# latentnetworks/vimure

Measured on AMD Instinct MI355X. Metric: CAVI iterations/sec (L=4 N=2000 M=200 K=2 synthetic, mutuality on), higher is better.
Workload: dtype f64

## Files before the change

vimure_amd/csrc/sweep_sl.hip:

```cpp
#include "sweep_sl.h"

#ifndef VMR_K
#error "compile with -DVMR_K=<number of categories>"
#endif
#ifndef SL_WPE
#define SL_WPE sl_wpe(2, false, true)
#endif

template <int K>
struct StepIn {
  double v[K];
  double w[K];
  unsigned cls, qt, tie;
  unsigned x0;
  unsigned e[sl_pf(K)];
};

template <int R> struct RC { static constexpr int value = R; };
template <class V> __device__ __forceinline__ const V* at_bytes(const V* p, unsigned off) {
  return reinterpret_cast<const V*>(reinterpret_cast<const char*>(p) + off);
}
template <class V> __device__ __forceinline__ V* at_bytes(V* p, unsigned off) {
  return reinterpret_cast<V*>(reinterpret_cast<char*>(p) + off);
}
__device__ __forceinline__ double rcp_nr2(double d) {
  double r = __builtin_amdgcn_rcp(d);
  r = fma(fma(-d, r, 1.0), r, r);
  return fma(fma(-d, r, 1.0), r, r);
}
#define SL_INL __attribute__((always_inline))
#ifndef SL_BATCH2
#define SL_BATCH2 8
#endif
template <int K> struct Batch { static constexpr int value = K <= 2 ? SL_BATCH2 : (K <= 4 ? 4 : 2); };

template <int K, bool UPDATE, bool ELBO, bool ALLFULL, bool STORE = true, bool DET = false, bool LPD = false>
__device__ __forceinline__ void sweep_body(const SlArgs& a, const Geo& g, const unsigned bx, const unsigned gx) {
  extern __shared__ __align__(16) unsigned char smem[];
  constexpr int PFK = sl_pf(K);
  constexpr bool LV0 = !UPDATE && !ELBO && !DET;
  constexpr bool LV0R = UPDATE && K >= 3;
  const int tid = threadIdx.x, lane = tid & 63, nthr = (int)blockDim.x;
  const int wv = __builtin_amdgcn_readfirstlane(tid >> 6), nw = nthr >> 6;
  const int Mp = g.Mp;
  const unsigned ytm = UPDATE ? (unsigned)a.yt * (unsigned)Mp : 0u;
  const unsigned hcm = a.do_hist ? (unsigned)a.hc * (unsigned)Mp : 0u;
  size_t off = 0;
  double* F = reinterpret_cast<double*>(smem + off); off += (size_t)ytm * K * 8;
  const int nHc = (int)hcm * K;
  double* Hc = reinterpret_cast<double*>(smem + off); off += (size_t)nHc * 8;
  double* Gth = reinterpret_cast<double*>(smem + off); off += (size_t)Mp * 8;
  double* Lth = reinterpret_cast<double*>(smem + off); off += UPDATE ? (size_t)Mp * 8 : 0;
  double* As = reinterpret_cast<double*>(smem + off); off += a.sum_a ? (size_t)Mp * K * 8 : 0;
  double* wsum = reinterpret_cast<double*>(smem + off); off += (size_t)g.W * 8;
  double* red = reinterpret_cast<double*>(smem + off); off += 16 * 8;
  double* xt = reinterpret_cast<double*>(smem + off); off += 64 * 8;
  double* lt = reinterpret_cast<double*>(smem + off); off += ELBO ? 256 * 8 : 0;
  double* EthL = reinterpret_cast<double*>(smem + off); off += a.rq ? (size_t)Mp * 8 : 0;
  const ParOff o = par_off(g.L, g.Mp, g.K);
  const int l = (int)bx / a.Gl, gb = (int)bx - l * a.Gl;
#ifdef SL_DEBUG
  unsigned long long* dbt = a.dbg_t ? a.dbg_t + ((size_t)bx * nw + wv) * 8 : nullptr;
  if (dbt && lane == 0) dbt[0] = wall_clock64();
#endif
  const size_t T = (size_t)g.N * g.N;
  const long long NS = (long long)((T + 63) / 64);
  const double gnu = a.par[o.sc + ((UPDATE || a.elbo_cur) ? SC_G_NU : SC_G_NU_STALE)];
  bool gz = false;
  for (int m = tid; m < Mp; m += nthr) {
    const double gv = a.par[o.G_th + (size_t)l * Mp + m];
    Gth[m] = gv;
    if (LV0 || LV0R) gz = gz || (m < g.M && gv == 0.0);
    if (UPDATE) Lth[m] = a.par[o.l_th + (size_t)l * Mp + m];
  }
  for (int q = tid; q < nHc; q += nthr) Hc[q] = 0.0;
  if (a.sum_a) for (int q = tid; q < Mp * K; q += nthr) As[q] = 0.0;
  if (a.rq) for (int m = tid; m < Mp; m += nthr) EthL[m] = m < g.M ? a.par[o.E_th + (size_t)l * Mp + m] : 0.0;
  if (UPDATE || ELBO) sp_math_tables(xt, lt, tid, nthr, ELBO);
  const double* lut = a.lutg + (size_t)l * g.W * 256;
  for (int w = tid; w < g.W; w += nthr) {
    double v = 0.0;
    for (int n = 0; n < 16; ++n) v += lut[(w * 16 + n) * 16 + 15];
    wsum[w] = v;
  }
  double Ela[K], Gla[K], Lla[K];
#pragma unroll
  for (int k = 0; k < K; ++k) { Ela[k] = a.par[o.E_la + l * K + k]; Gla[k] = a.par[o.G_la + l * K + k]; Lla[k] = a.par[o.l_la + l * K + k]; if (LV0 || LV0R) gz = gz || Gla[k] == 0.0; }
  const double eps = g.eps;
  const double sc_h = DET ? __builtin_amdgcn_ldexp(1.0, g.det_sh) : 0.0, sc_r = DET ? __builtin_amdgcn_ldexp(1.0, g.det_shr) : 0.0;
  const double sc_a = DET ? __builtin_amdgcn_ldexp(1.0, DET_SH_A) : 0.0;
  auto fxm = [](double v, double scale) SL_INL -> unsigned long long {
    return (unsigned long long)(__double_as_longlong(fma(v, scale, 6755399441055744.0)) - 0x4338000000000000ll);
  };
  auto lds_add = [&](double* p, double v, double scale) SL_INL {
    if (DET) atomicAdd(reinterpret_cast<unsigned long long*>(p), fxm(v, scale)); else atomicAdd(p, v);
  };
  const float rcp_mp = 1.0f / (float)Mp, hrcp_mp = 0.5f * rcp_mp;
  auto row_level = [&](unsigned ym) SL_INL -> unsigned { return (unsigned)__builtin_fmaf((float)ym, rcp_mp, hrcp_mp); };
  const double lp0_0 = log(1.0 + eps), lp0_k = log(eps);
  double e_lin = 0.0, e_q = 0.0, e_log = 0.0;
  double accF[K], acc0[K];
#pragma unroll
  for (int k = 0; k < K; ++k) { accF[k] = 0.0; acc0[k] = 0.0; }
  unsigned long long ie_lin = 0ull, ie_q = 0ull, ie_log = 0ull, iaccF[K];
#pragma unroll
  for (int k = 0; k < K; ++k) iaccF[k] = 0ull;
  double* Hl = a.Hg + ((size_t)l * NH + (gb % NH)) * g.Y * Mp * K;
  auto det_H = [&]() SL_INL { return a.det + (size_t)l * g.Y * Mp * K; };
  auto det_A = [&]() SL_INL { return a.det + (size_t)g.L * g.Y * Mp * K + (size_t)l * g.W * 64 * K; };
  auto det_F = [&]() SL_INL { return a.det + (size_t)g.L * g.Y * Mp * K + (size_t)g.L * g.W * 64 * K + (size_t)l * K; };
  auto det_R = [&]() SL_INL { return a.det + (size_t)g.L * g.Y * Mp * K + (size_t)g.L * g.W * 64 * K + (size_t)g.L * K; };
  const unsigned* rsl = a.rs + (size_t)l * (NS + 1);
  const unsigned* syl = a.sy + (size_t)l * NS;
  const unsigned* El = a.E + a.ebase[l];
  const unsigned* pl = (a.rm2 ? a.rm2 : a.perm) + (size_t)l * NS * 64;
  const uint8_t* cl = ALLFULL ? nullptr : a.cls + (size_t)l * T;
  const unsigned* Ql = a.Qt ? a.Qt + (size_t)l * T : nullptr;
  const uint64_t* Rl = a.Rb ? a.Rb + (size_t)l * T * g.W : nullptr;
  double* rl = a.rho + (size_t)l * T * K;
  double* rho_slack = a.rho + (size_t)g.L * T * K;
  const double* lpl = a.logpr + (size_t)l * T * K;
  constexpr bool LPDV = LPD && K == 2 && UPDATE && !ELBO;
  const double* lpdl = LPDV ? a.lpd + (size_t)l * T : nullptr;
  const double lpb0 = (K == 2 && UPDATE) ? a.lpb[2 * l] : 0.0, lpb1 = (K == 2 && UPDATE) ? a.lpb[2 * l + 1] : 0.0;
  const unsigned* rql = a.rq ? a.rq + (size_t)l * (T + 1) : nullptr;
  const unsigned short* Rml = a.rq ? a.Rm + a.rbase[l] : nullptr;
  const unsigned lim_y = UPDATE ? (a.do_hist ? (unsigned)min(a.yt, a.hc) : (unsigned)a.yt) : (a.do_hist ? (unsigned)a.hc : 0xffffffffu);
  const unsigned lim1 = (UPDATE && a.yt < g.Y) ? (unsigned)a.yt : 0xffffffffu;
  const unsigned lim2 = (a.do_hist && a.hc < g.Y) ? (unsigned)a.hc : 0xffffffffu;

  const long long Gl_ = a.Gl;
  unsigned* tick = reinterpret_cast<unsigned*>(smem + off); off += 16;
  if (tid == 0) { tick[0] = 2u * (unsigned)nw; tick[1] = 0u; }
  auto step_of = [&](unsigned t) SL_INL -> long long { return (long long)gb + (long long)t * Gl_; };
  auto draw = [&]() SL_INL -> long long {
    unsigned t = 0u;
    if (lane == 0) t = atomicAdd(tick, 1u);
    return step_of((unsigned)__builtin_amdgcn_readfirstlane((int)t));
  };
  long long s = step_of((unsigned)wv), sn = step_of((unsigned)(nw + wv));
  unsigned ea = 0;
  int R = 0;
  unsigned ymax = 0;
  unsigned rgv = 0;
  StepIn<K> P;

  const unsigned lane4 = (unsigned)lane * 4u, laneK8 = (unsigned)lane * (unsigned)(K * 8);
  const unsigned T32 = (unsigned)T;
  auto fetch_range = [&](long long st) SL_INL {
    const unsigned ra = rsl[st + (lane < 1 ? 0 : 1)], ry = syl[st];
    rgv = lane == 2 ? ry : ra;
  };
  auto fetch_tie = [&](StepIn<K>& d, long long st, const bool lp_const = false) SL_INL {
    const size_t row0 = (size_t)st * 64;
    const bool ok = (unsigned)row0 + (unsigned)lane < T32;
    d.qt = 0u; d.tie = 0u;
    if (ALLFULL) d.cls = ok ? 1u : 0u;
    else {
      const unsigned c = (unsigned)*at_bytes(cl + row0, (unsigned)lane);
      d.cls = ok ? c : 0u;
      d.tie = *at_bytes(pl + row0, lane4);
    }
    if (ELBO && Ql) d.qt = *at_bytes(Ql + row0, lane4);
    d.x0 = 0u;
    if (LV0 && a.x0p) d.x0 = *at_bytes(a.x0p + (size_t)l * NS * 64 + row0, lane4);
#pragma unroll
    for (int k = 0; k < K; ++k) { d.v[k] = 0.0; d.w[k] = 0.0; }
    if (LPDV) {
      if (lp_const) d.v[0] = lp0_k - lp0_0;
      else d.v[0] = *at_bytes(lpdl + row0, (unsigned)lane * 8u);
    } else if (UPDATE || ELBO) {
      if (lp_const) {
#pragma unroll
        for (int k = 0; k < K; ++k) d.v[k] = k == 0 ? lp0_0 : lp0_k;
      } else load_k<K>(at_bytes(lpl + row0 * K, laneK8), d.v);
    }
    if (!UPDATE && a.do_hist != 2) load_k<K>(at_bytes(static_cast<const double*>(rl) + row0 * K, laneK8), d.w);
  };
  auto fetch_ent = [&](StepIn<K>& d, unsigned base, auto cntc) SL_INL {
    constexpr int CNT = decltype(cntc)::value;
    const unsigned* pe = El + base;
#pragma unroll
    for (int j = 0; j < CNT; ++j) d.e[j] = *at_bytes(pe + j * 64, lane4);
  };

  if (s < NS) {
    ea = rsl[s];
    R = (int)((rsl[s + 1] - ea) >> 6);
    ymax = syl[s];
    fetch_range(sn < NS ? sn : s);
    fetch_tie(P, s);
    fetch_ent(P, ea, RC<PFK>{});
  }
#ifdef SL_DEBUG
  if (dbt && lane == 0) dbt[4] = wall_clock64();
#endif
  __builtin_amdgcn_s_waitcnt(0x0F70);
  bool lv0_off = false;
  if (LV0 || LV0R) lv0_off = __syncthreads_or(gz ? 1 : 0) != 0;
  else __syncthreads();
#ifdef SL_DEBUG
  if (dbt && lane == 0) dbt[5] = wall_clock64();
#endif
  const double gnu_f = a.par[o.sc + (a.nu_stale ? SC_G_NU_STALE : SC_G_NU)];
  if (UPDATE) {
    for (int q = tid; q < (int)ytm; q += nthr) {
      const int y = q / Mp, m = q - y * Mp;
#pragma unroll
      for (int k = 0; k < K; ++k) F[q * K + k] = (m < g.M) ? f_entry(g.mut, Lth[m], Gth[m], Lla[k], Gla[k], gnu_f, y) : 0.0;
    }
    __syncthreads();
  }
  double Tfull = 0.0;
  for (int w = 0; w < g.W; ++w) Tfull += wsum[w];
#ifdef SL_DEBUG
  if (dbt && lane == 0) dbt[1] = wall_clock64();
#endif

  auto add_lists = [&](unsigned t, bool on, const double (&rr)[K]) SL_INL {
    if (a.rm2) {
#pragma unroll
      for (int h_ = 0; h_ < 2; ++h_) {
        const unsigned m = h_ ? (t >> 16) : (t & 0xffffu);
        const bool v = on && m != 0xffffu;
        const unsigned long long vm = __ballot(v);
        if (vm == 0ull) continue;
        const int m0 = __builtin_amdgcn_readlane((int)m, __builtin_ctzll(vm));
        if (__all(!v || (int)m == m0)) {
#pragma unroll
          for (int k = 0; k < K; ++k) {
            const double sm_ = wave_sum(v ? rr[k] : 0.0);
            if (lane == 0) lds_add(&As[m0 * K + k], sm_, sc_a);
          }
        } else if (v) {
#pragma unroll
          for (int k = 0; k < K; ++k) lds_add(&As[m * K + k], rr[k], sc_a);
        }
      }
      return;
    }
    unsigned q0 = 0, q1 = 0;
    if (on) { q0 = rql[t]; q1 = rql[t + 1]; }
    for (unsigned i = 0;; ++i) {
      const bool v = q0 + i < q1;
      const unsigned long long vm = __ballot(v);
      if (vm == 0ull) break;
      const int m = v ? (int)Rml[q0 + i] : -1;
      const int m0 = __builtin_amdgcn_readlane(m, __builtin_ctzll(vm));
      if (__all(!v || m == m0)) {
#pragma unroll
        for (int k = 0; k < K; ++k) {
          const double sm_ = wave_sum(v ? rr[k] : 0.0);
          if (lane == 0) lds_add(&As[m0 * K + k], sm_, sc_a);
        }
      } else if (v) {
#pragma unroll
        for (int k = 0; k < K; ++k) lds_add(&As[m * K + k], rr[k], sc_a);
      }
    }
  };
  auto mask_sum = [&](unsigned cls, unsigned tie) SL_INL -> double {
    if (ALLFULL) return Tfull;
    double Tt = 0.0;
    if (cls == 1u) Tt = Tfull;
    else if (cls == 2u && a.rm2) {
      const unsigned m0 = tie & 0xffffu, m1 = tie >> 16;
      Tt = (m0 != 0xffffu ? EthL[m0] : 0.0) + (m1 != 0xffffu ? EthL[m1] : 0.0);
    } else if (cls == 2u && rql) {
      const unsigned q0 = rql[tie], q1 = rql[tie + 1];
      for (unsigned q = q0; q < q1; ++q) Tt += EthL[Rml[q]];
    } else if (cls == 2u) {
      const uint64_t* rwt = Rl + (size_t)tie * g.W;
      for (int w = 0; w < g.W; ++w) {
        uint64_t bits = rwt[w];
        if (bits == ~0ull) { Tt += wsum[w]; continue; }
        for (int n = 0; bits != 0; ++n, bits >>= 4) Tt += lut[((w * 16 + n) << 4) + (unsigned)(bits & 15u)];
      }
    }
    return Tt;
  };
  const double gnu_cur = a.par[o.sc + SC_G_NU];
  auto w2_at = [&](unsigned ym, int k) SL_INL -> double {
    const unsigned y = row_level(ym);
    const double z2 = gnu_cur * (double)y, den = Gth[ym - y * (unsigned)Mp] * Gla[k] + z2;
    return (y == 0u || den == 0.0) ? 0.0 : z2 / den;
  };
  auto f_far = [&](unsigned ym, double (&f)[K]) SL_INL {
    const unsigned y = row_level(ym);
    const unsigned m = ym - y * (unsigned)Mp;
    const double lt = Lth[m], gt = Gth[m];
#pragma unroll
    for (int k = 0; k < K; ++k) f[k] = f_entry(g.mut, lt, gt, Lla[k], Gla[k], gnu_f, (int)y);
  };
  auto elbo_inner = [&](unsigned ent, const double (&er)[2]) SL_INL -> double {
    const unsigned ym = SL_YM(ent);
    const unsigned y = row_level(ym);
    const double z2 = gnu * (double)y, gt = Gth[ym - y * (unsigned)Mp];
    const double inner = fma(gt, er[0], z2 * er[1]);
    return (SL_INR(ent) ? inner : 0.0) + eps;
  };
  auto walk1_near = [&](const unsigned* e, auto npc, double (&U)[K]) SL_INL {
    constexpr int NP = decltype(npc)::value, BT = Batch<K>::value;
#pragma unroll
    for (int j0 = 0; j0 < NP; j0 += BT) {
      double f[BT][K];
#pragma unroll
      for (int u = 0; u < BT; ++u) {
        if (j0 + u < NP) {
#pragma unroll
          for (int k = 0; k < K; ++k) f[u][k] = F[SL_YM(e[j0 + u]) * K + k];
        }
      }
#pragma unroll
      for (int u = 0; u < BT; ++u) {
        if (j0 + u < NP) {
          const double dx = (double)SL_X(e[j0 + u]);
#pragma unroll
          for (int k = 0; k < K; ++k) U[k] = fma(dx, f[u][k], U[k]);
        }
      }
    }
  };
  auto walk2_near = [&](const unsigned* e, auto npc, const double (&r)[K], const double (&er)[2]) SL_INL {
#ifndef SL_LG
#define SL_LG 2
#endif
    constexpr int NP = decltype(npc)::value, LG = SL_LG;
#pragma unroll
    for (int j0 = 0; j0 < NP; j0 += LG) {
      double in_[LG];
#pragma unroll
      for (int u = 0; u < LG; ++u) {
        if (j0 + u < NP) {
          const unsigned ym = SL_YM(e[j0 + u]);
          const double dx = (double)SL_X(e[j0 + u]);
          if (a.do_hist) {
#pragma unroll
            for (int k = 1; k < K; ++k) lds_add(&Hc[(unsigned)k * hcm + ym], dx * r[k], sc_h);
          }
          if (ELBO) in_[u] = elbo_inner(e[j0 + u], er);
        }
      }
      if (ELBO) {
#pragma unroll
        for (int u = 0; u < LG; ++u) if (j0 + u < NP) {
          const double term = (double)SL_X(e[j0 + u]) * log_tab(in_[u], lt);
          if (DET) ie_log += fxm(term, sc_r); else e_log += term;
        }
        __builtin_amdgcn_sched_barrier(0);
      }
    }
  };
  auto deficit = [&](unsigned ent, double dfc) SL_INL {
    lds_add(&Hc[SL_YM(ent)], (double)SL_X(ent) * dfc, sc_h);
  };
  auto compute = [&](auto rct, const StepIn<K>& cur, const size_t row0, const bool act, const unsigned ea_c, const int Rr, const unsigned sy_word) SL_INL {
    const unsigned ymax = sy_word & 0xffffu, nf = a.farl ? sy_word >> 16 : 0x7fffffffu;
    const unsigned n1 = (LV0 && a.h0s && !lv0_off) ? sy_word >> 16 : 0x7fffffffu;
    constexpr int RCT = decltype(rct)::value;
    constexpr int NP = RCT < 0 ? PFK : RCT;
    const unsigned cls = cur.cls, qt = cur.qt, tie = cur.tie;
    const unsigned* pe = El + ea_c;
    auto rounds = [&](auto gbc, auto&& use, const int Rr) SL_INL {
      constexpr int GB = decltype(gbc)::value;
      unsigned rg[PFK];
#pragma unroll
      for (int i = 0; i < PFK; ++i) rg[i] = i < Rr ? cur.e[i] : 0u;
      for (int j0 = 0; j0 < Rr; j0 += PFK) {
#pragma unroll
        for (int gi = 0; gi < PFK; gi += GB) {
          unsigned c[GB];
#pragma unroll
          for (int u = 0; u < GB; ++u) {
            c[u] = rg[gi + u];
            const int jn = j0 + gi + u + PFK;
            rg[gi + u] = *at_bytes(jn < Rr ? pe + (size_t)jn * 64 : a.Ez, lane4);
          }
          if (j0 + gi < Rr) use(c, (unsigned)(j0 + gi));
        }
      }
    };
    double r[K], er[2] = {0.0, 0.0};
#pragma unroll
    for (int k = 0; k < K; ++k) r[k] = act ? cur.w[k] : 0.0;
    if (a.do_hist == 2) {
#pragma unroll
      for (int k = 0; k < K; ++k) r[k] = (k == 1) ? 1.0 : 0.0;
    }
    double Tt = 0.0;
    if (UPDATE || ELBO) Tt = mask_sum(cls, tie);
    double dfc = 0.0;
    bool irr = false;

    if (UPDATE) {
      double U[K];
#pragma unroll
      for (int k = 0; k < K; ++k) U[k] = 0.0;
#ifdef SL_DEBUG
      if (g.dbg & 16) {} else
#endif
      if (RCT >= 0) walk1_near(cur.e, RC<NP>{}, U);
      else {
        constexpr int GB = Batch<K>::value < 4 ? Batch<K>::value : 4;
        const unsigned n1u = (LV0R && a.lv0r && !lv0_off) ? sy_word >> 16 : 0x7fffffffu;
        double sl0 = 0.0, sx1 = 0.0;
        rounds(RC<GB>{}, [&](const unsigned (&c)[GB], const unsigned j) SL_INL {
          if (LV0R && j >= n1u) {
            double l0[GB];
#pragma unroll
            for (int u = 0; u < GB; ++u) l0[u] = Lth[SL_YM(c[u])];
#pragma unroll
            for (int u = 0; u < GB; ++u) { const double dx = (double)SL_X(c[u]); sl0 = fma(dx, l0[u], sl0); sx1 += dx; }
            return;
          }
          if (ymax < lim1 || j >= nf) { walk1_near(c, RC<GB>{}, U); return; }
          double f[GB][K];
          bool fr[GB];
#pragma unroll
          for (int u = 0; u < GB; ++u) {
            const unsigned ym = SL_YM(c[u]);
            fr[u] = ym >= ytm;
#pragma unroll
            for (int k = 0; k < K; ++k) f[u][k] = F[(fr[u] ? 0u : ym) * K + k];
          }
#pragma unroll
          for (int u = 0; u < GB; ++u) {
            const double dx = fr[u] ? 0.0 : (double)SL_X(c[u]);
#pragma unroll
            for (int k = 0; k < K; ++k) U[k] = fma(dx, f[u][k], U[k]);
          }
#pragma unroll
          for (int u = 0; u < GB; ++u) {
            if (__any(fr[u])) {
              if (fr[u]) {
                double ff[K];
                f_far(SL_YM(c[u]), ff);
                const double dx = (double)SL_X(c[u]);
#pragma unroll
                for (int k = 0; k < K; ++k) U[k] = fma(dx, ff[k], U[k]);
              }
            }
          }
        }, Rr);
        if (LV0R && a.lv0r && !lv0_off) {
#pragma unroll
          for (int k = 0; k < K; ++k) U[k] += fma(Lla[k], sx1, sl0);
        }
      }
      double aa[K];
      bool done = false;
      if (K == 2) {
        double c[K];
#pragma unroll
        for (int k = 0; k < K; ++k) c[k] = fma(-Tt, Ela[k], U[k]);
        const double d = ((LPDV ? cur.v[0] : cur.v[K - 1] - cur.v[0]) + c[K - 1]) - c[0];
        bool safe = fabs(c[0]) + lpb0 < 700.0 && fabs(c[K - 1]) + lpb1 < 700.0 && fabs(d) < 700.0;
        if (!__all(safe)) {
          double v[K];
#pragma unroll
          for (int k = 0; k < K; ++k) v[k] = cur.v[k];
          if (LPDV) load_k<K>(at_bytes(lpl + row0 * K, laneK8), v);
#pragma unroll
          for (int k = 0; k < K; ++k) aa[k] = v[k] + c[k];
          safe = fabs(aa[0]) < 700.0 && fabs(aa[K - 1]) < 700.0 && fabs(d) < 700.0;
        }
        if (__all(safe)) {
          const double e = exp_tab(d, xt);
          r[0] = rcp_nr2(1.0 + e);
          r[K - 1] = e * r[0];
          done = true;
        }
      } else {
#pragma unroll
        for (int k = 0; k < K; ++k) aa[k] = (cur.v[k] + U[k]) - Tt * Ela[k];
      }
      if (!done) {
        double sum = 0.0;
        bool tame = true;
#pragma unroll
        for (int k = 0; k < K; ++k) tame = tame && fabs(aa[k]) < 700.0;
        tame = __all(tame);
        if (tame) {
#pragma unroll
          for (int k = 0; k < K; ++k) r[k] = exp_tab(aa[k], xt);
        } else {
#pragma unroll
          for (int k = 0; k < K; ++k) r[k] = exp(aa[k]);
        }
#pragma unroll
        for (int k = 0; k < K; ++k) sum += r[k];
        if (sum > 0.0) {
#pragma unroll
          for (int k = 0; k < K; ++k) r[k] /= sum;
        }
        if (a.do_hist) {
          double sm = 0.0;
#pragma unroll
          for (int k = 0; k < K; ++k) sm += r[k];
          dfc = 1.0 - sm;
          if (fabs(dfc) <= 1e-14 || !act) dfc = 0.0;
          irr = __any(dfc != 0.0);
          if (irr && lane == 0) tick[1] = 1u;
        }
      }
      if (STORE) store_k<K>(act ? at_bytes(rl + row0 * K, laneK8) : at_bytes(rho_slack, laneK8), r);
      if (act && (ALLFULL || cls == 1u)) {
#pragma unroll
        for (int k = 0; k < K; ++k) { if (DET) iaccF[k] += fxm(r[k], sc_a); else accF[k] += r[k]; }
      }
      if (!ALLFULL && a.sum_a) add_lists(tie, act && cls == 2u, r);
    } else if (a.do_hist) {
      double sm = 0.0;
#pragma unroll
      for (int k = 0; k < K; ++k) sm += r[k];
      dfc = 1.0 - sm;
      if (fabs(dfc) <= 1e-14 || !act) dfc = 0.0;
      irr = __any(dfc != 0.0);
      if (irr && lane == 0) tick[1] = 1u;
      if (!ELBO && a.do_hist == 1 && act && (ALLFULL || cls == 1u)) {
#pragma unroll
        for (int k = 0; k < K; ++k) { if (DET) iaccF[k] += fxm(r[k], sc_a); else accF[k] += r[k]; }
      }
      if (!ALLFULL && !ELBO && a.sum_a) add_lists(tie, act && cls == 2u, r);
    }
    if (ELBO) {
#pragma unroll
      for (int k = 0; k < K; ++k) { const double ek = exp_tab(r[k], xt); er[0] = fma(ek, Gla[k], er[0]); er[1] += ek; }
    }
#ifdef SL_DEBUG
    if (g.dbg & 32) {} else
#endif
    if (a.do_hist || ELBO) {
      if (RCT >= 0) {
        walk2_near(cur.e, RC<NP>{}, r, er);
        if (irr) {
#pragma unroll
          for (int j = 0; j < NP; ++j) deficit(cur.e[j], dfc);
        }
      } else {
        const bool skip0 = LV0 && a.x0p != nullptr && a.do_hist == 1 && n1 != 0x7fffffffu && !irr;
        const int Rw = skip0 ? min(Rr, (int)n1) : Rr;
        double sx0 = skip0 ? (double)cur.x0 : 0.0;
        rounds(RC<1>{}, [&](const unsigned (&c1)[1], const unsigned j) SL_INL {
          const unsigned c = c1[0], ym = SL_YM(c), x = SL_X(c);
          const bool far_round = j < nf && lim2 != 0xffffffffu;
          const bool fr = far_round && ym >= hcm;
          const double dx = (double)x;
          if (LV0 && a.do_hist && j >= n1) {
            sx0 += dx;
            if (irr) lds_add(&Hc[ym], dx * dfc, sc_h);
          } else if (a.do_hist) {
            if (!fr) {
              if (!(skip0 && ym < (unsigned)Mp)) {
#pragma unroll
                for (int k = 1; k < K; ++k) lds_add(&Hc[(unsigned)k * hcm + ym], dx * r[k], sc_h);
              }
              if (irr) lds_add(&Hc[ym], dx * dfc, sc_h);
            }
            if (far_round && !a.farl && __any(fr)) {
              if (fr && x != 0u) {
                if (DET) {
                  unsigned long long* d0 = a.det;
                  asm volatile("" : "+s"(d0));
                  unsigned long long* d = d0 + (size_t)l * g.Y * Mp * K + (size_t)ym * K;
#pragma unroll
                  for (int k = 1; k < K; ++k) atomicAdd(&d[k], fxm((double)x * r[k], sc_h));
                  if (dfc != 0.0) atomicAdd(&d[0], fxm((double)x * dfc, sc_h));
                } else {
                  double* d = Hl + (size_t)ym * K;
#pragma unroll
                  for (int k = 1; k < K; ++k) atomicAdd(&d[k], (double)x * r[k]);
                  if (dfc != 0.0) atomicAdd(&d[0], (double)x * dfc);
                }
              }
              asm volatile("" ::: "memory");
            }
          }
          if (ELBO) { const double term = (double)x * log_tab(elbo_inner(c, er), lt); if (DET) ie_log += fxm(term, sc_r); else e_log += term; }
        }, Rw);
        if (LV0 && a.h0s && a.do_hist == 1 && act) {
#pragma unroll
          for (int k = 1; k < K; ++k) acc0[k] = fma(r[k], sx0, acc0[k]);
        }
      }
    }
    if (ELBO && act) {
      double sr = 0.0, se = 0.0, en = 0.0;
#pragma unroll
      for (int k = 0; k < K; ++k) {
        sr += r[k]; se += r[k] * Ela[k];
        en += r[k] * cur.v[k] - r[k] * log_tab(r[k] + eps, lt);
      }
      if (DET) { ie_lin += det_fx(en - se * Tt, g.det_shr); if (Ql) ie_q += det_fx(sr * (double)qt, g.det_shr); }
      else { e_lin += en - se * Tt; if (Ql) e_q += sr * (double)qt; }
    }
  };
  auto body = [&](auto rct) SL_INL {
    constexpr int RCT = decltype(rct)::value;
    constexpr int NP = RCT < 0 ? PFK : RCT;
    const size_t row0 = (size_t)s * 64;
    const bool act = (unsigned)row0 + (unsigned)lane < T32;
    const unsigned ea_c = ea;
    const int Rr = RCT < 0 ? R : RCT;
    const StepIn<K> cur = P;
    const long long s2 = sn, s3 = draw();
    const bool more = s2 < NS;
    const unsigned ea2 = more ? (unsigned)__builtin_amdgcn_readlane((int)rgv, 0) : ea_c;
    const int R2 = more ? (int)(((unsigned)__builtin_amdgcn_readlane((int)rgv, 1) - ea2) >> 6) : 0;
    const unsigned ym2 = more ? (unsigned)__builtin_amdgcn_readlane((int)rgv, 2) : 0u;
    fetch_range(s3 < NS ? s3 : s);
    fetch_tie(P, more ? s2 : s, RCT == 0 && a.lp0 != 0);
    if (RCT >= 0 || PFK <= 8) fetch_ent(P, ea2, RC<NP>{});
    else {
      const unsigned* pe = El + ea2;
#pragma unroll
      for (int j0 = 0; j0 < PFK; j0 += 8) {
        if (j0 == 0 || j0 < R2) {
#pragma unroll
          for (int j = j0; j < j0 + 8; ++j) P.e[j] = *at_bytes(pe + j * 64, lane4);
        }
      }
    }
    compute(rct, cur, row0, act, ea_c, Rr, ymax);
    constexpr int NST = (UPDATE && STORE) ? (K % 2 == 0 ? K / 2 : K) : 0;
    static_assert(NST <= 8, "vmcnt immediate below");
    if (RCT >= 0) __builtin_amdgcn_s_waitcnt(0x0F70 | NST);
    else __builtin_amdgcn_s_waitcnt(0x0F70);
    s = s2; sn = s3; ea = ea2; R = R2; ymax = ym2;
  };
  auto run = [&](auto rct) SL_INL {
    constexpr int RCT = decltype(rct)::value;
    do { body(rct); } while (s < NS && R == RCT && (ymax & 0xffffu) < lim_y);
  };
  while (s < NS) {
    if (R > SL_PF || (ymax & 0xffffu) >= lim_y) { body(RC<-1>{}); continue; }
    switch (R) {
      case 0: run(RC<0>{}); break;
      case 1: run(RC<1>{}); break;
      case 2: run(RC<2>{}); break;
      case 3: run(RC<3>{}); break;
      case 4: run(RC<4>{}); break;
      case 5: run(RC<5>{}); break;
      case 6: run(RC<6>{}); break;
      case 7: run(RC<7>{}); break;
      default: run(RC<8>{}); break;
    }
  }

#ifdef SL_DEBUG
  if (dbt && lane == 0) dbt[2] = wall_clock64();
#endif
  const bool nu_here = a.nu_acc && a.do_hist == 1;
  if (nu_here) asm volatile("s_waitcnt vmcnt(0)" ::: "memory");
  __syncthreads();
  if (nu_here) {
    double a0p = 0.0;
    for (int q = (tick[1] ? 0 : (int)hcm) + tid; q < nHc; q += nthr) {
      const double v = DET ? det_back(reinterpret_cast<const unsigned long long*>(Hc)[q], g.det_sh) : Hc[q];
      if (v != 0.0) {
        const int k = q / (int)hcm;
        const unsigned ym = (unsigned)(q - k * (int)hcm);
        a0p += ((k ? w2_at(ym, k) : 0.0) - w2_at(ym, 0)) * v;
      }
    }
    a0p = block_sum_n(a0p, red);
    if (tid == 0) {
      if (DET) atomicAdd(&det_R()[4], det_fx(a0p, g.det_sh)); else atomicAdd(&a.nu_acc[0], a0p);
    }
  }
#ifdef SL_DEBUG
  if (dbt && lane == 0) dbt[6] = wall_clock64();
#endif
  const int f0 = (nu_here && nw > 1) ? 64 : 0;
#ifdef SL_DEBUG
  if (g.dbg & 8) {} else
#endif
  if (a.do_hist && tid >= f0) {
    for (int q = (tick[1] ? 0 : (int)hcm) + tid - f0; q < nHc; q += nthr - f0) {
      if (DET) {
        const unsigned long long iv = reinterpret_cast<const unsigned long long*>(Hc)[q];
        if (iv != 0ull) { const int k = q / (int)hcm, ym = q - k * (int)hcm; atomicAdd(&det_H()[(size_t)ym * K + k], iv); }
        continue;
      }
      const double v = Hc[q];
      if (v != 0.0) {
        const int k = q / (int)hcm, ym = q - k * (int)hcm;
        atomicAdd(&Hl[(size_t)ym * K + k], v);
      }
    }
  }
  if (a.sum_a && tid >= f0) {
    double* out = a.slotA + ((size_t)l * NSLOT + (gb % NSLOT)) * (size_t)g.W * 64 * K;
    for (int q = tid - f0; q < g.M * K; q += nthr - f0) {
      if (DET) { const unsigned long long iv = reinterpret_cast<const unsigned long long*>(As)[q]; if (iv != 0ull) atomicAdd(&det_A()[q], iv); continue; }
      const double v = As[q];
      if (v != 0.0) atomicAdd(&out[q], v);
    }
  }
#ifdef SL_DEBUG
  if (dbt && lane == 0) dbt[7] = wall_clock64();
#endif
  if (nu_here) {
    __shared__ int nu_last;
    if (tid == 0) {
      asm volatile("s_waitcnt vmcnt(0)" ::: "memory");
      const double t = atomicAdd(&a.nu_acc[1], 1.0);
      nu_last = (t == (double)(gx - 1u));
      if (nu_last) __builtin_amdgcn_fence(__ATOMIC_ACQUIRE, "agent");
      asm volatile("s_waitcnt vmcnt(0)" ::: "memory");
    }
    __syncthreads();
    if (nu_last && a.farl) {
      if (tid == 0) a.nu_acc[1] = 0.0;
    } else if (nu_last) {
      double far = 0.0;
      const size_t hcs = (size_t)g.Y * Mp * K;
      const int y0 = max(1, a.hc);
      if (a.hc < g.Y) {
        for (int ll = 0; ll < g.L; ++ll) {
          const double* H0 = a.Hg + (size_t)ll * NH * hcs;
          const double* gthl = a.par + o.G_th + (size_t)ll * Mp;
          for (int it = y0 * Mp + tid; it < g.Y * Mp; it += nthr) {
            const int y = it / Mp, m = it - y * Mp;
            double v0[NH], vk[NH][K > 1 ? K - 1 : 1];
#pragma unroll
            for (int c = 0; c < NH; ++c) {
              v0[c] = H0[(size_t)c * hcs + (size_t)it * K];
#pragma unroll
              for (int k = 1; k < K; ++k) vk[c][k - 1] = H0[(size_t)c * hcs + (size_t)it * K + k];
            }
            if (DET) {
              const unsigned long long* hi = a.det + (size_t)ll * hcs + (size_t)it * K;
              v0[0] += det_back(hi[0], g.det_sh);
#pragma unroll
              for (int k = 1; k < K; ++k) vk[0][k - 1] += det_back(hi[k], g.det_sh);
            }
            double h_[K];
#pragma unroll
            for (int k = 0; k < K; ++k) h_[k] = 0.0;
#pragma unroll
            for (int c = 0; c < NH; ++c) {
              h_[0] += v0[c];
#pragma unroll
              for (int k = 1; k < K; ++k) h_[k] += vk[c][k - 1];
            }
            bool any = h_[0] != 0.0;
#pragma unroll
            for (int k = 1; k < K; ++k) any = any || h_[k] != 0.0;
            if (any && m < g.M) {
              const double z2 = gnu_cur * (double)y, gt = gthl[m];
              const double d0 = gt * a.par[o.G_la + ll * K] + z2, w0 = d0 == 0.0 ? 0.0 : z2 / d0;
              far -= w0 * h_[0];
#pragma unroll
              for (int k = 1; k < K; ++k) {
                const double dk = gt * a.par[o.G_la + ll * K + k] + z2;
                far += ((dk == 0.0 ? 0.0 : z2 / dk) - w0) * h_[k];
              }
            }
          }
        }
      }
      far = block_sum_n(far, red);
      if (tid == 0) {
        double tot = far;
        if (DET) { unsigned long long* dR = det_R(); tot += det_back(atomicAdd(&dR[4], 0ull), g.det_sh); dR[4] = 0ull; } else tot += atomicAdd(&a.nu_acc[0], 0.0);
        for (int ll = 0; ll < g.L; ++ll) tot += a.nu_acc[2 + ll];
        a.nu_acc[0] = 0.0; a.nu_acc[1] = 0.0;
        a.elbo_dev[1] = tot;
        if (a.commit_nu) {
          double* sc = const_cast<double*>(a.par) + o.sc;
          sc[SC_G_NU_STALE] = sc[SC_G_NU];
          sc[SC_NU_SHP] = sc[SC_A_ETA] + tot;
          sc[SC_G_NU] = exp(digamma_pos(sc[SC_NU_SHP]) - log(sc[SC_NU_RTE]));
          sc[SC_E_NU] = sc[SC_NU_SHP] / sc[SC_NU_RTE];
        }
      }
    }
  }
  auto wave_isum = [&](unsigned long long v) SL_INL -> unsigned long long {
#pragma unroll
    for (int o2 = 32; o2 > 0; o2 >>= 1) {
      const unsigned lo = (unsigned)__shfl_xor((int)(unsigned)v, o2, 64), hi = (unsigned)__shfl_xor((int)(unsigned)(v >> 32), o2, 64);
      v += ((unsigned long long)hi << 32) | lo;
    }
    return v;
  };
  if ((UPDATE || (!ELBO && a.do_hist == 1)) && a.slotF) {
#pragma unroll
    for (int k = 0; k < K; ++k) {
      if (DET) { const unsigned long long v = wave_isum(iaccF[k]); if (lane == 0 && v != 0ull) atomicAdd(&det_F()[k], v); continue; }
      double v = block_sum_n(accF[k], red);
      if (tid == 0) atomicAdd(&a.slotF[((size_t)l * NSLOT + (gb % NSLOT)) * K + k], v);
    }
  }
  if (LV0 && a.h0s && a.do_hist == 1) {
#pragma unroll
    for (int k = 1; k < K; ++k) {
      const double v = block_sum_n(acc0[k], red);
      if (tid == 0 && v != 0.0) atomicAdd(&a.h0s[((size_t)l * NSLOT + (gb % NSLOT)) * K + k], v);
    }
  }
  if (ELBO) {
    if (DET) {
      const unsigned long long v1 = wave_isum(ie_lin), v2 = wave_isum(ie_log), v3 = wave_isum(ie_q);
      if (lane == 0) { unsigned long long* dR = det_R(); atomicAdd(&dR[1], v1); atomicAdd(&dR[2], v2); atomicAdd(&dR[3], v3); }
    } else {
      double v1 = block_sum_n(e_lin, red);
      double v2 = block_sum_n(e_log, red);
      double v3 = block_sum_n(e_q, red);
      if (tid == 0) {
        double* out = a.slotR + (size_t)(bx % NSLOT) * 4;
        atomicAdd(&out[1], v1); atomicAdd(&out[2], v2); atomicAdd(&out[3], v3);
      }
    }
  }
#ifdef SL_DEBUG
  if (dbt && lane == 0) dbt[3] = wall_clock64();
#endif
}

#define SL_BOUNDS(K, UPDATE, ELBO, ALLFULL) \
  __launch_bounds__(sl_tpb_max(K, ELBO, ALLFULL, UPDATE), (K == 2 && !ELBO && ALLFULL) ? SL_WPE : sl_wpe(K, ELBO, ALLFULL, UPDATE))
template <int K, bool UPDATE, bool ELBO, bool ALLFULL, bool STORE = true, bool DET = false, bool LPD = false>
__global__ SL_BOUNDS(K, UPDATE, ELBO, ALLFULL) void k_sweep_sl(SlArgs a, Geo g) {
  sweep_body<K, UPDATE, ELBO, ALLFULL, STORE, DET, LPD>(a, g, blockIdx.x, gridDim.x);
}
template <int K, bool UPDATE, bool ELBO, bool ALLFULL, bool STORE = true, bool LPD = false>
__global__ __launch_bounds__(sl_tpb_max_b(K, ELBO, ALLFULL), sl_wpe_b(K, ELBO, ALLFULL)) void k_sweep_sl_b(const SlUnit* __restrict__ units, const int* __restrict__ blk_unit) {
  const SlUnit& u = units[blk_unit[blockIdx.x]];
  sweep_body<K, UPDATE, ELBO, ALLFULL, STORE, false, LPD>(u.a, u.g, blockIdx.x - (unsigned)u.blk0, (unsigned)u.nblk);
}

template <bool UPDATE, bool ELBO, bool ALLFULL, bool STORE = true, bool DET = false, bool LPD = false>
static int sl_launch_one_(vmr_ctx* h, const SlShape& sh, SlArgs& a) {
  constexpr int K = VMR_K;
  const Geo& g = h->g;
  const long long NS = ((long long)g.N * g.N + 63) / 64, nw = sh.tpb / 64;
  int rc = grid_per_layer(h, k_sweep_sl<K, UPDATE, ELBO, ALLFULL, STORE, DET, LPD>, sh.smem, &a.Gl, (NS + nw - 1) / nw, sh.tpb);
  if (rc) return rc;
#ifdef SL_DEBUG
  static unsigned long long* dbg_buf = nullptr;
  const char* tf = h->opt.debug_times[0] ? h->opt.debug_times : nullptr;
  const size_t nwv = (size_t)g.L * a.Gl * nw;
  a.dbg_t = nullptr;
  if (tf) {
    if (!dbg_buf) (void)hipMalloc(&dbg_buf, (size_t)1 << 22);
    if (nwv * 64 <= ((size_t)1 << 22)) a.dbg_t = dbg_buf;
  }
#endif
  hipLaunchKernelGGL((k_sweep_sl<K, UPDATE, ELBO, ALLFULL, STORE, DET, LPD>), dim3(g.L * a.Gl), dim3(sh.tpb), sh.smem, h->stream, a, g);
#ifdef SL_DEBUG
  if (a.dbg_t) {
    std::vector<unsigned long long> t(nwv * 8);
    (void)hipStreamSynchronize(h->stream);
    (void)hipMemcpy(t.data(), dbg_buf, nwv * 64, hipMemcpyDeviceToHost);
    if (FILE* f = fopen(tf, "a")) {
      fprintf(f, "launch %d%d hist %d waves %zu tpb %d\n", (int)UPDATE, (int)ELBO, a.do_hist, nwv, sh.tpb);
      for (size_t i = 0; i < nwv; ++i) fprintf(f, "%llu %llu %llu %llu %llu %llu %llu %llu\n", t[i * 8], t[i * 8 + 1], t[i * 8 + 2], t[i * 8 + 3], t[i * 8 + 4], t[i * 8 + 5], t[i * 8 + 6], t[i * 8 + 7]);
      fclose(f);
    }
  }
#endif
  return VMR_OK;
}

template <bool UPDATE, bool ELBO, bool ALLFULL, bool STORE = true, bool DET = false>
static int sl_launch_one(vmr_ctx* h, const SlShape& sh, SlArgs& a) {
  if (VMR_K == 2 && UPDATE && !ELBO && a.lpd) return sl_launch_one_<UPDATE, ELBO, ALLFULL, STORE, DET, VMR_K == 2 && UPDATE && !ELBO>(h, sh, a);
  return sl_launch_one_<UPDATE, ELBO, ALLFULL, STORE, DET>(h, sh, a);
}

#define SL_CAT2(a, b) a##b
#define SL_CAT(a, b) SL_CAT2(a, b)
int SL_CAT(vmr_sl_launch_k, VMR_K)(vmr_ctx* h, int mode, const SlShape& sh, SlArgs& a) {
  if (a.det) {
    if (a.cls == nullptr) {
      switch (mode) {
        case 0: return sl_launch_one<true, false, true, true, true>(h, sh, a);
        case 4: return sl_launch_one<true, false, true, false, true>(h, sh, a);
        case 1: return sl_launch_one<true, true, true, true, true>(h, sh, a);
        case 2: return sl_launch_one<false, true, true, true, true>(h, sh, a);
        default: return sl_launch_one<false, false, true, true, true>(h, sh, a);
      }
    }
    switch (mode) {
      case 0: return sl_launch_one<true, false, false, true, true>(h, sh, a);
      case 4: return sl_launch_one<true, false, false, false, true>(h, sh, a);
      case 1: return sl_launch_one<true, true, false, true, true>(h, sh, a);
      case 2: return sl_launch_one<false, true, false, true, true>(h, sh, a);
      default: return sl_launch_one<false, false, false, true, true>(h, sh, a);
    }
  }
  if (a.cls == nullptr) {
    switch (mode) {
      case 0: return sl_launch_one<true, false, true>(h, sh, a);
      case 1: return sl_launch_one<true, true, true>(h, sh, a);
      case 2: return sl_launch_one<false, true, true>(h, sh, a);
      case 4: return sl_launch_one<true, false, true, false>(h, sh, a);
      default: return sl_launch_one<false, false, true>(h, sh, a);
    }
  }
  switch (mode) {
    case 0: return sl_launch_one<true, false, false>(h, sh, a);
    case 1: return sl_launch_one<true, true, false>(h, sh, a);
    case 2: return sl_launch_one<false, true, false>(h, sh, a);
    case 4: return sl_launch_one<true, false, false, false>(h, sh, a);
    default: return sl_launch_one<false, false, false>(h, sh, a);
  }
}

template <bool UPDATE, bool ELBO, bool ALLFULL, bool STORE = true, bool LPD = false>
static int sl_launch_batch_one_(vmr_ctx* h, hipStream_t st, const SlUnit* units, const int* blk_unit, int nblocks, int tpb, size_t smem) {
  constexpr int K = VMR_K;
  if (smem > 48 * 1024)
    HIPCHK(h, hipFuncSetAttribute(reinterpret_cast<const void*>(k_sweep_sl_b<K, UPDATE, ELBO, ALLFULL, STORE, LPD>), hipFuncAttributeMaxDynamicSharedMemorySize, (int)smem));
  hipLaunchKernelGGL((k_sweep_sl_b<K, UPDATE, ELBO, ALLFULL, STORE, LPD>), dim3(nblocks), dim3(tpb), smem, st, units, blk_unit);
  return VMR_OK;
}
template <bool UPDATE, bool ELBO, bool ALLFULL, bool STORE = true>
static int sl_launch_batch_one(vmr_ctx* h, hipStream_t st, bool lpd, const SlUnit* units, const int* blk_unit, int nblocks, int tpb, size_t smem) {
  if (VMR_K == 2 && UPDATE && !ELBO && lpd) return sl_launch_batch_one_<UPDATE, ELBO, ALLFULL, STORE, VMR_K == 2 && UPDATE && !ELBO>(h, st, units, blk_unit, nblocks, tpb, smem);
  return sl_launch_batch_one_<UPDATE, ELBO, ALLFULL, STORE>(h, st, units, blk_unit, nblocks, tpb, smem);
}
int SL_CAT(vmr_sl_launch_batch_k, VMR_K)(vmr_ctx* h, hipStream_t st, int mode, int allfull, const SlUnit* units, const int* blk_unit, int nblocks,
                                          int tpb, size_t smem) {
  const bool lpd = h->lpd != nullptr;
  if (mode == 3) return allfull ? sl_launch_batch_one<false, false, true>(h, st, lpd, units, blk_unit, nblocks, tpb, smem)
                                : sl_launch_batch_one<false, false, false>(h, st, lpd, units, blk_unit, nblocks, tpb, smem);
  if (mode == 4) return allfull ? sl_launch_batch_one<true, false, true, false>(h, st, lpd, units, blk_unit, nblocks, tpb, smem)
                                : sl_launch_batch_one<true, false, false, false>(h, st, lpd, units, blk_unit, nblocks, tpb, smem);
  if (allfull) return mode ? sl_launch_batch_one<true, true, true>(h, st, lpd, units, blk_unit, nblocks, tpb, smem)
                           : sl_launch_batch_one<true, false, true>(h, st, lpd, units, blk_unit, nblocks, tpb, smem);
  return mode ? sl_launch_batch_one<true, true, false>(h, st, lpd, units, blk_unit, nblocks, tpb, smem)
              : sl_launch_batch_one<true, false, false>(h, st, lpd, units, blk_unit, nblocks, tpb, smem);
}
```

Baseline: 6060.

## Store K=2 F table as difference plane and skip second gather when bounded

For K=2 update sweeps, the LDS F table is stored as two planes, f1-f0 and f0, instead of interleaved pairs. The near walk gathers only the difference plane plus the x count. A precomputed bound on Lth magnitude gives an x-sum limit under which the exp-safety check is guaranteed, so the f0 plane is gathered only when that bound fails. This roughly halves LDS reads in the hot walk, at the cost of a block-wide max reduction, extra branches, and a redundant second walk whenever the bound is not met.

```diff
diff --git a/vimure_amd/csrc/sweep_sl.hip b/vimure_amd/csrc/sweep_sl.hip
--- a/vimure_amd/csrc/sweep_sl.hip
+++ b/vimure_amd/csrc/sweep_sl.hip
@@ -29,6 +29,23 @@
   return fma(fma(-d, r, 1.0), r, r);
 }
 #define SL_INL __attribute__((always_inline))
+__device__ __forceinline__ void f_pair(int mut, double lth, double gth, const double* lla, const double* gla, double gnu, int y, double& f0, double& fd) {
+#pragma clang fp contract(off)
+  double f[2];
+#pragma unroll
+  for (int k = 0; k < 2; ++k) {
+    double w = 1.0;
+    if (mut) {
+      const double z1 = gth * gla[k], z2 = gnu * (double)y;
+      double den = z1 + z2;
+      den = (den == 0.0) ? 1.0 : den;
+      w = z1 / den;
+    }
+    f[k] = (lth + lla[k]) * w;
+  }
+  f0 = f[0];
+  fd = f[1] - f[0];
+}
 #ifndef SL_BATCH2
 #define SL_BATCH2 8
 #endif
@@ -39,6 +56,7 @@
   extern __shared__ __align__(16) unsigned char smem[];
   constexpr int PFK = sl_pf(K);
   constexpr bool LV0 = !UPDATE && !ELBO && !DET;
+  constexpr bool FD = UPDATE && K == 2;
   constexpr bool LV0R = UPDATE && K >= 3;
   const int tid = threadIdx.x, lane = tid & 63, nthr = (int)blockDim.x;
   const int wv = __builtin_amdgcn_readfirstlane(tid >> 6), nw = nthr >> 6;
@@ -131,7 +149,8 @@
 
   const long long Gl_ = a.Gl;
   unsigned* tick = reinterpret_cast<unsigned*>(smem + off); off += 16;
-  if (tid == 0) { tick[0] = 2u * (unsigned)nw; tick[1] = 0u; }
+  unsigned long long* fmx = reinterpret_cast<unsigned long long*>(tick + 2);
+  if (tid == 0) { tick[0] = 2u * (unsigned)nw; tick[1] = 0u; if (FD) *fmx = 0ull; }
   auto step_of = [&](unsigned t) SL_INL -> long long { return (long long)gb + (long long)t * Gl_; };
   auto draw = [&]() SL_INL -> long long {
     unsigned t = 0u;
@@ -206,13 +225,31 @@
   if (UPDATE) {
     for (int q = tid; q < (int)ytm; q += nthr) {
       const int y = q / Mp, m = q - y * Mp;
-#pragma unroll
-      for (int k = 0; k < K; ++k) F[q * K + k] = (m < g.M) ? f_entry(g.mut, Lth[m], Gth[m], Lla[k], Gla[k], gnu_f, y) : 0.0;
+      if (FD) {
+        double f0 = 0.0, fd = 0.0;
+        if (m < g.M) f_pair(g.mut, Lth[m], Gth[m], Lla, Gla, gnu_f, y, f0, fd);
+        F[q] = fd; F[ytm + q] = f0;
+      } else {
+#pragma unroll
+        for (int k = 0; k < K; ++k) F[q * K + k] = (m < g.M) ? f_entry(g.mut, Lth[m], Gth[m], Lla[k], Gla[k], gnu_f, y) : 0.0;
+      }
+    }
+    if (FD) {
+      double lm = 0.0;
+      for (int m = tid; m < g.M; m += nthr) lm = fmax(lm, fabs(Lth[m]));
+      if (lm > 0.0) atomicMax(fmx, (unsigned long long)__double_as_longlong(lm));
     }
     __syncthreads();
   }
+  const double Lthm = FD ? __longlong_as_double((long long)*fmx) : 0.0;
+  const double Fm0 = Lthm + fabs(Lla[0]), Fm1 = Lthm + fabs(Lla[K - 1]);
   double Tfull = 0.0;
   for (int w = 0; w < g.W; ++w) Tfull += wsum[w];
+  unsigned xs_lim = 0u;
+  if (FD) {
+    const double x0_ = (700.0 - fma(Tfull, fabs(Ela[0]), lpb0)) / Fm0, x1_ = (700.0 - fma(Tfull, fabs(Ela[K - 1]), lpb1)) / Fm1;
+    xs_lim = (unsigned)__builtin_amdgcn_readfirstlane((int)(unsigned)(fmin(x0_, x1_) * (1.0 - 1e-9)));
+  }
 #ifdef SL_DEBUG
   if (dbt && lane == 0) dbt[1] = wall_clock64();
 #endif
@@ -279,7 +316,7 @@
     }
     return Tt;
   };
-  const double gnu_cur = a.par[o.sc + SC_G_NU];
+  double gnu_cur = FD ? 0.0 : a.par[o.sc + SC_G_NU];
   auto w2_at = [&](unsigned ym, int k) SL_INL -> double {
     const unsigned y = row_level(ym);
     const double z2 = gnu_cur * (double)y, den = Gth[ym - y * (unsigned)Mp] * Gla[k] + z2;
@@ -289,9 +326,11 @@
     const unsigned y = row_level(ym);
     const unsigned m = ym - y * (unsigned)Mp;
     const double lt = Lth[m], gt = Gth[m];
+    if (FD) { f_pair(g.mut, lt, gt, Lla, Gla, gnu_f, (int)y, f[0], f[K - 1]); return; }
 #pragma unroll
     for (int k = 0; k < K; ++k) f[k] = f_entry(g.mut, lt, gt, Lla[k], Gla[k], gnu_f, (int)y);
   };
+  auto f_at = [&](unsigned ym, int k) SL_INL -> double { return FD ? F[(k == 0 ? ytm : 0u) + ym] : F[ym * K + k]; };
   auto elbo_inner = [&](unsigned ent, const double (&er)[2]) SL_INL -> double {
     const unsigned ym = SL_YM(ent);
     const unsigned y = row_level(ym);
@@ -308,7 +347,7 @@
       for (int u = 0; u < BT; ++u) {
         if (j0 + u < NP) {
 #pragma unroll
-          for (int k = 0; k < K; ++k) f[u][k] = F[SL_YM(e[j0 + u]) * K + k];
+          for (int k = 0; k < K; ++k) f[u][k] = f_at(SL_YM(e[j0 + u]), k);
         }
       }
 #pragma unroll
@@ -318,6 +357,19 @@
 #pragma unroll
           for (int k = 0; k < K; ++k) U[k] = fma(dx, f[u][k], U[k]);
         }
+      }
+    }
+  };
+  auto walk1_plane = [&](const unsigned* e, auto npc, const unsigned plane, double& S, unsigned& Xs) SL_INL {
+    constexpr int NP = decltype(npc)::value, BT = Batch<K>::value;
+#pragma unroll
+    for (int j0 = 0; j0 < NP; j0 += BT) {
+      double f[BT];
+#pragma unroll
+      for (int u = 0; u < BT; ++u) if (j0 + u < NP) f[u] = *at_bytes(F, SL_YM(e[j0 + u]) * 8u + plane);
+#pragma unroll
+      for (int u = 0; u < BT; ++u) {
+        if (j0 + u < NP) { const unsigned x = SL_X(e[j0 + u]); S = fma((double)x, f[u], S); Xs += x; }
       }
     }
   };
@@ -335,8 +387,11 @@
           const unsigned ym = SL_YM(e[j0 + u]);
           const double dx = (double)SL_X(e[j0 + u]);
           if (a.do_hist) {
-#pragma unroll
-            for (int k = 1; k < K; ++k) lds_add(&Hc[(unsigned)k * hcm + ym], dx * r[k], sc_h);
+            if (FD) lds_add(at_bytes(Hc + hcm, ym * 8u), dx * r[K - 1], sc_h);
+            else {
+#pragma unroll
+              for (int k = 1; k < K; ++k) lds_add(&Hc[(unsigned)k * hcm + ym], dx * r[k], sc_h);
+            }
           }
           if (ELBO) in_[u] = elbo_inner(e[j0 + u], er);
         }
@@ -396,10 +451,13 @@
       double U[K];
 #pragma unroll
       for (int k = 0; k < K; ++k) U[k] = 0.0;
+      double Ud = 0.0;
+      unsigned Xs = 0u;
 #ifdef SL_DEBUG
       if (g.dbg & 16) {} else
 #endif
-      if (RCT >= 0) walk1_near(cur.e, RC<NP>{}, U);
+      if (RCT >= 0 && FD) walk1_plane(cur.e, RC<NP>{}, 0u, Ud, Xs);
+      else if (RCT >= 0) walk1_near(cur.e, RC<NP>{}, U);
       else {
         constexpr int GB = Batch<K>::value < 4 ? Batch<K>::value : 4;
         const unsigned n1u = (LV0R && a.lv0r && !lv0_off) ? sy_word >> 16 : 0x7fffffffu;
@@ -414,6 +472,23 @@
             return;
           }
           if (ymax < lim1 || j >= nf) { walk1_near(c, RC<GB>{}, U); return; }
+          if (FD) {
+#pragma unroll
+            for (int u = 0; u < GB; ++u) {
+              const unsigned ym = SL_YM(c[u]);
+              const bool fr1 = ym >= ytm;
+              double f1[K];
+#pragma unroll
+              for (int k = 0; k < K; ++k) f1[k] = f_at(fr1 ? 0u : ym, k);
+              if (__any(fr1)) {
+                if (fr1) f_far(ym, f1);
+              }
+              const double dx = (double)SL_X(c[u]);
+#pragma unroll
+              for (int k = 0; k < K; ++k) U[k] = fma(dx, f1[k], U[k]);
+            }
+            return;
+          }
           double f[GB][K];
           bool fr[GB];
 #pragma unroll
@@ -450,19 +525,36 @@
       double aa[K];
       bool done = false;
       if (K == 2) {
+        const double cd = fma(-Tt, Ela[K - 1] - Ela[0], RCT >= 0 ? Ud : U[K - 1]);
+        const double d = (LPDV ? cur.v[0] : cur.v[K - 1] - cur.v[0]) + cd;
+        bool safe = fabs(d) < 700.0;
+        bool exact = RCT < 0;
+        if (RCT >= 0) {
+          safe = safe && Xs < xs_lim;
+          if (!__all(safe)) {
+            unsigned xs_ = 0u;
+            walk1_plane(cur.e, RC<NP>{}, ytm * 8u, U[0], xs_);
+            exact = true;
+          }
+        }
         double c[K];
 #pragma unroll
-        for (int k = 0; k < K; ++k) c[k] = fma(-Tt, Ela[k], U[k]);
-        const double d = ((LPDV ? cur.v[0] : cur.v[K - 1] - cur.v[0]) + c[K - 1]) - c[0];
-        bool safe = fabs(c[0]) + lpb0 < 700.0 && fabs(c[K - 1]) + lpb1 < 700.0 && fabs(d) < 700.0;
-        if (!__all(safe)) {
-          double v[K];
-#pragma unroll
-          for (int k = 0; k < K; ++k) v[k] = cur.v[k];
-          if (LPDV) load_k<K>(at_bytes(lpl + row0 * K, laneK8), v);
-#pragma unroll
-          for (int k = 0; k < K; ++k) aa[k] = v[k] + c[k];
-          safe = fabs(aa[0]) < 700.0 && fabs(aa[K - 1]) < 700.0 && fabs(d) < 700.0;
+        for (int k = 0; k < K; ++k) c[k] = 0.0;
+        if (exact) {
+          double tt = Tt;
+          if (RCT >= 0) asm volatile("" : "+v"(tt));
+          c[0] = fma(-tt, Ela[0], U[0]);
+          c[K - 1] = c[0] + cd;
+          safe = fabs(c[0]) + lpb0 < 700.0 && fabs(c[K - 1]) + lpb1 < 700.0 && fabs(d) < 700.0;
+          if (!__all(safe)) {
+            double v[K];
+#pragma unroll
+            for (int k = 0; k < K; ++k) v[k] = cur.v[k];
+            if (LPDV) load_k<K>(at_bytes(lpl + row0 * K, laneK8), v);
+#pragma unroll
+            for (int k = 0; k < K; ++k) aa[k] = v[k] + c[k];
+            safe = fabs(aa[0]) < 700.0 && fabs(aa[K - 1]) < 700.0 && fabs(d) < 700.0;
+          }
         }
         if (__all(safe)) {
           const double e = exp_tab(d, xt);
@@ -650,6 +742,7 @@
 #ifdef SL_DEBUG
   if (dbt && lane == 0) dbt[2] = wall_clock64();
 #endif
+  if (FD) gnu_cur = a.par[o.sc + SC_G_NU];
   const bool nu_here = a.nu_acc && a.do_hist == 1;
   if (nu_here) asm volatile("s_waitcnt vmcnt(0)" ::: "memory");
   __syncthreads();
```

Result: no change. 6106 (median of 6 runs) (+0.8%).
